# zhvng/open-musiclm

Hardware: NVIDIA H100
Metric: coarse-stage training tokens/sec (positions fed to the transformer per optimiser step / step time) (higher is better)
Workload: dtype bf16 (fp16 operands for the forward GEMMs on LayerNorm outputs x weights; fp32 accumulate)

## Files before the change

### open-musiclm_b200/csrc/attn_bwd_tc.cu

```cuda
#include "common.cuh"
#include "ptx.cuh"
#include "../../include/omlm_b200.h"
#include <stdlib.h>

namespace omlm {

constexpr int kBtThreads = 384;
constexpr int kBtBQ = 64, kBtBK = 128;
constexpr float kBtL2e = 1.4426950408889634f;

constexpr int kBoK = 0, kBoV = 16384, kBoQ = 32768 , kBoDO = 49152 ;
constexpr int kBoP = 65536 , kBoDS = 81920 , kBoBar = 98304 ;
constexpr int kBoSds = 98368;
constexpr int kBtMaxSmem = 232448;
constexpr int kBtSdsLd = 72;
constexpr int kBoWin = kBoSds + 2 * 64 * kBtSdsLd * 4;

static int bt_win_ld(int h) { return ((62 + h) / h + 64 + 23) / 32 * 32 + 8; }

__device__ __forceinline__ float bt_ex2(float x) {
  float y;
  asm("ex2.approx.ftz.f32 %0, %1;" : "=f"(y) : "f"(x));
  return y;
}
__device__ __forceinline__ void bt_red2(float* addr, float a, float b) {
  asm volatile("red.global.add.v2.f32 [%0], {%1, %2};" ::"l"(addr), "f"(a), "f"(b) : "memory");
}

__device__ __forceinline__ int bt_ld_acquire(const int* p) {
  int v;
  asm volatile("ld.acquire.gpu.global.b32 %0, [%1];" : "=r"(v) : "l"(p) : "memory");
  return v;
}
__device__ __forceinline__ unsigned long long bt_globaltimer() {
  unsigned long long t;
  asm volatile("mov.u64 %0, %%globaltimer;" : "=l"(t));
  return t;
}
__device__ __noinline__ void bt_wait_turn(const int* ctr, int turn, int* err) {
  const unsigned long long t0 = bt_globaltimer();
  while (bt_ld_acquire(ctr) != turn) {
    if (*reinterpret_cast<volatile int*>(err) != 0) return;
    if (bt_globaltimer() - t0 > 4000000000ull) { atomicExch(err, 1); return; }
    __nanosleep(64);
  }
}
__device__ __forceinline__ void bt_pass_turn(int* ctr) {
  asm volatile("red.release.gpu.global.add.s32 [%0], 1;" ::"l"(ctr) : "memory");
}

struct BtDet {
  int* turn_dq;
  int* turn_kv;
  int* meta;
  int* err;
  float* dpart;
};

template <bool DET>
__global__ void __launch_bounds__(kBtThreads, 1)
attn_bwd_tc_kernel(const __grid_constant__ CUtensorMap tmQ, const __grid_constant__ CUtensorMap tmDO,
                   const __grid_constant__ CUtensorMap tmKV, const float* __restrict__ lse2, const float* __restrict__ dsum,
                   const float* __restrict__ table, int table_ld, const unsigned char* __restrict__ key_mask,
                   float* __restrict__ dqn, float* __restrict__ dkvn, float* __restrict__ dtable, int N, int h, float scale,
                   int Wacc, int win_ld, int tiles_per_chunk, int nbatch, const BtDet det) {
  extern __shared__ __align__(1024) uint8_t smem_raw[];
  uint8_t* smem = smem_raw + ((1024u - (smem_u32(smem_raw) & 1023u)) & 1023u);
  uint64_t* bars = reinterpret_cast<uint64_t*>(smem + kBoBar);
  uint64_t* kv_full = bars + 0;
  uint64_t* qd_full = bars + 1;
  uint64_t* qd_empty = bars + 3;
  float* dacc = reinterpret_cast<float*>(smem + kBoWin) + 2 * h * win_ld;

  const int wg = threadIdx.x >> 7, lane = threadIdx.x & 31;
  const int R = N * h;
  const int n_rt = (R + kBtBQ - 1) / kBtBQ;
  const int n_kt = (N + kBtBK - 1) / kBtBK;
  const int b = blockIdx.x % nbatch;
  int u = blockIdx.x / nbatch, kt = 0;
  for (; kt < n_kt; ++kt) {
    const int cnt = (n_rt - (kt * kBtBK * h) / kBtBQ + tiles_per_chunk - 1) / tiles_per_chunk;
    if (u < cnt) break;
    u -= cnt;
  }
  const int j0 = kt * kBtBK;
  const int rt0 = (j0 * h) / kBtBQ + u * tiles_per_chunk;
  const int rt1 = min(n_rt, rt0 + tiles_per_chunk);
  const int T = rt1 - rt0;
  const int i_lo = (rt0 * kBtBQ) / h, i_hi = min(N - 1, (rt1 * kBtBQ - 1) / h);
  const int dmin = max(0, i_lo - j0 - (kBtBK - 1));
  const int wacc_used = i_hi - j0 - dmin + 1;

  if (threadIdx.x == 0) {
    tma_prefetch_desc(&tmQ); tma_prefetch_desc(&tmDO); tma_prefetch_desc(&tmKV);
    mbar_init(kv_full, 1);
    for (int i = 0; i < 2; ++i) { mbar_init(&qd_full[i], 1); mbar_init(&qd_empty[i], 2); }
    fence_barrier_init();
  }
  for (int x = threadIdx.x; x < 2 * h * Wacc; x += blockDim.x) dacc[x] = 0.f;
  __syncthreads();

  if (wg == 0) {
    asm volatile("setmaxnreg.dec.sync.aligned.u32 40;");
    if (threadIdx.x == 0) {
      mbar_expect_tx(kv_full, 2 * 16384);
      tma_load_2d(smem + kBoK, &tmKV, kv_full, 0, b * N + j0);
      tma_load_2d(smem + kBoV, &tmKV, kv_full, 64, b * N + j0);
      for (int t = 0; t < T; ++t) {
        const int st = t & 1;
        mbar_wait(&qd_empty[st], ((t >> 1) & 1) ^ 1);
        mbar_expect_tx(&qd_full[st], 2 * 8192);
        tma_load_2d(smem + kBoQ + st * 8192, &tmQ, &qd_full[st], 0, b * R + (rt0 + t) * kBtBQ);
        tma_load_2d(smem + kBoDO + st * 8192, &tmDO, &qd_full[st], 0, b * R + (rt0 + t) * kBtBQ);
      }
    }
  } else {
    asm volatile("setmaxnreg.inc.sync.aligned.u32 232;");
    const int cw = wg - 1;
    const int wq = (threadIdx.x >> 5) & 3, qr = lane >> 2, qc = lane & 3;
    const bool leader = (threadIdx.x & 127) == 0;
    const int kbase = j0 + cw * 64;
    const uint32_t sk = smem_u32(smem + kBoK) + cw * 8192, sv = smem_u32(smem + kBoV) + cw * 8192;
    uint8_t* p_tile = smem + kBoP + cw * 8192;
    uint8_t* ds_tile = smem + kBoDS + cw * 8192;
    float* sdsf = reinterpret_cast<float*>(smem + kBoSds) + cw * 64 * kBtSdsLd;
    float* win = reinterpret_cast<float*>(smem + kBoWin) + cw * h * win_ld;
    float* wacc = dacc + cw * h * Wacc;
    const int tid128 = threadIdx.x & 127;
    const uint32_t sp = smem_u32(p_tile), sds = smem_u32(ds_tile);
    const float sc2 = scale * kBtL2e;
    uint32_t vis = 0;
#pragma unroll
    for (int c = 0; c < 8; ++c)
#pragma unroll
      for (int e = 0; e < 2; ++e) {
        const int j = kbase + 8 * c + 2 * qc + e;
        if (j < N && (key_mask == nullptr || key_mask[static_cast<long long>(b) * N + j] != 0)) vis |= 1u << (2 * c + e);
      }
    float dv[32], dk[32];
#pragma unroll
    for (int x = 0; x < 32; ++x) { dv[x] = 0.f; dk[x] = 0.f; }
    mbar_wait(kv_full, 0);
    for (int t = 0; t < T; ++t) {
      const int st = t & 1;
      const int rbase = (rt0 + t) * kBtBQ;
      const uint32_t sq = smem_u32(smem + kBoQ + st * 8192), sdo = smem_u32(smem + kBoDO + st * 8192);
      mbar_wait(&qd_full[st], (t >> 1) & 1);
      float s[32], dp[32];
      wgmma_fence();
#pragma unroll
      for (int ks = 0; ks < 4; ++ks) {
        Wgmma<64, false>::ss<0, 0>(s, make_smem_desc(sq + ks * 32, 16, 1024), make_smem_desc(sk + ks * 32, 16, 1024), ks > 0 ? 1u : 0u);
        Wgmma<64, false>::ss<0, 0>(dp, make_smem_desc(sdo + ks * 32, 16, 1024), make_smem_desc(sv + ks * 32, 16, 1024), ks > 0 ? 1u : 0u);
      }
      wgmma_commit();
      const int it_lo = min(rbase, R - 1) / h, it_hi = min(rbase + kBtBQ - 1, R - 1) / h;
      {
        const int win_w = it_hi - it_lo + 64, dlo = it_lo - kbase - 63;
        for (int x = tid128; x < h * win_w; x += 128) {
          const int hh = x / win_w, w = x - hh * win_w, d = dlo + w;
          win[hh * win_ld + w] = d >= 0 ? __ldg(table + hh * static_cast<long>(table_ld) + d) * kBtL2e : 0.f;
        }
      }
      asm volatile("bar.sync %0, 128;" ::"r"(1 + cw) : "memory");
      wgmma_wait<0>();
      wgmma_reg_fence(s);
      wgmma_reg_fence(dp);
#pragma unroll
      for (int hr = 0; hr < 2; ++hr) {
        const int lr = wq * 16 + qr + hr * 8;
        const int r = rbase + lr;
        const bool row_ok = r < R;
        const int rc = min(r, R - 1);
        const int i = rc / h, hh = rc - i * h;
        const float lse = lse2[static_cast<long long>(b) * R + rc];
        const float D = dsum[static_cast<long long>(b) * R + rc];
        const float* wrow = win + hh * win_ld + i - it_lo + 63 - 2 * qc;
        const int dcol = i - kbase - 2 * qc;
        uint8_t* prow = p_tile + lr * 128;
        uint8_t* drow = ds_tile + lr * 128;
#pragma unroll
        for (int c = 0; c < 8; ++c) {
          float pp[2], dd[2];
#pragma unroll
          for (int e = 0; e < 2; ++e) {
            const bool live = row_ok && ((vis >> (2 * c + e)) & 1u) && dcol >= 8 * c + e;
            const float x = s[4 * c + 2 * hr + e];
            pp[e] = live ? bt_ex2(fmaf(x, sc2, wrow[-8 * c - e]) - lse) : 0.f;
            dd[e] = pp[e] * (dp[4 * c + 2 * hr + e] - D);
          }
          *reinterpret_cast<float2*>(sdsf + lr * kBtSdsLd + 8 * c + 2 * qc) = make_float2(dd[0], dd[1]);
          const uint32_t off = static_cast<uint32_t>(((c ^ (lr & 7)) << 4) + 4 * qc);
          *reinterpret_cast<uint32_t*>(prow + off) = pack_bf16x2(pp[0], pp[1]);
          *reinterpret_cast<uint32_t*>(drow + off) = pack_bf16x2(dd[0], dd[1]);
        }
      }
      fence_proxy_async();
      asm volatile("bar.sync %0, 128;" ::"r"(1 + cw) : "memory");
      float dq[32];
      wgmma_fence();
#pragma unroll
      for (int ks = 0; ks < 4; ++ks) {
        Wgmma<64, false>::ss<1, 1>(dv, make_smem_desc(sp + ks * 2048, 8192, 1024), make_smem_desc(sdo + ks * 2048, 8192, 1024), 1u);
        Wgmma<64, false>::ss<1, 1>(dk, make_smem_desc(sds + ks * 2048, 8192, 1024), make_smem_desc(sq + ks * 2048, 8192, 1024), 1u);
        Wgmma<64, false>::ss<0, 1>(dq, make_smem_desc(sds + ks * 32, 16, 1024), make_smem_desc(sk + ks * 2048, 8192, 1024), ks > 0 ? 1u : 0u);
      }
      wgmma_commit();
      {
        const int dlo = max(0, it_lo - kbase - 63), dhi = it_hi - kbase;
        const int W = dhi - dlo + 1;
        for (int p = tid128; p < h * W; p += 128) {
          const int hh = p / W, dl = dlo + (p - hh * W);
          const int i0 = max((rbase - hh + h - 1) / h, kbase + dl);
          const int i1 = min(min((rbase + kBtBQ - 1 - hh) / h, N - 1), kbase + dl + 63);
          float sum = 0.f;
          for (int i = i0; i <= i1; ++i) sum += sdsf[(i * h + hh - rbase) * kBtSdsLd + (i - dl - kbase)];
          wacc[hh * Wacc + dl - dmin] += sum;
        }
      }
      wgmma_wait<0>();
      wgmma_reg_fence(dq);
      wgmma_reg_fence(dv);
      wgmma_reg_fence(dk);
      asm volatile("bar.sync %0, 128;" ::"r"(1 + cw) : "memory");
      if (leader) mbar_arrive(&qd_empty[st]);
      int* turn = DET ? det.turn_dq + static_cast<long>(b) * n_rt + rt0 + t : nullptr;
      if constexpr (DET) {
        if (leader) bt_wait_turn(turn, 2 * kt + cw, det.err);
        asm volatile("bar.sync %0, 128;" ::"r"(1 + cw) : "memory");
      }
#pragma unroll
      for (int hr = 0; hr < 2; ++hr) {
        const int r = rbase + wq * 16 + qr + hr * 8;
        if (r < R) {
          float* dst = dqn + (static_cast<long long>(b) * R + r) * 64 + 2 * qc;
#pragma unroll
          for (int c = 0; c < 8; ++c) bt_red2(dst + 8 * c, dq[4 * c + 2 * hr] * scale, dq[4 * c + 2 * hr + 1] * scale);
        }
      }
      if constexpr (DET) {
        __threadfence();
        asm volatile("bar.sync %0, 128;" ::"r"(1 + cw) : "memory");
        if (leader) bt_pass_turn(turn);
      }
    }
    int* kv_turn = DET ? det.turn_kv + (static_cast<long>(b) * n_kt + kt) * 2 + cw : nullptr;
    if constexpr (DET) {
      if (leader) bt_wait_turn(kv_turn, u, det.err);
      asm volatile("bar.sync %0, 128;" ::"r"(1 + cw) : "memory");
    }
#pragma unroll
    for (int hr = 0; hr < 2; ++hr) {
      const int j = kbase + wq * 16 + qr + hr * 8;
      if (j < N) {
        float* dst = dkvn + (static_cast<long long>(b) * N + j) * 128 + 2 * qc;
#pragma unroll
        for (int c = 0; c < 8; ++c) {
          bt_red2(dst + 8 * c, dk[4 * c + 2 * hr] * scale, dk[4 * c + 2 * hr + 1] * scale);
          bt_red2(dst + 64 + 8 * c, dv[4 * c + 2 * hr], dv[4 * c + 2 * hr + 1]);
        }
      }
    }
    if constexpr (DET) {
      __threadfence();
      asm volatile("bar.sync %0, 128;" ::"r"(1 + cw) : "memory");
      if (leader) bt_pass_turn(kv_turn);
    }
    asm volatile("bar.sync 3, 256;" ::: "memory");
    if constexpr (DET) {
      float* up = det.dpart + static_cast<long>(blockIdx.x) * h * Wacc;
      for (int x = threadIdx.x - 128; x < h * wacc_used; x += 256) {
        const int hh = x / wacc_used, w = x - hh * wacc_used;
        up[hh * Wacc + w] = dacc[hh * Wacc + w] + dacc[(h + hh) * Wacc + w];
      }
      if (threadIdx.x == 128) { det.meta[2 * blockIdx.x] = dmin; det.meta[2 * blockIdx.x + 1] = wacc_used; }
    } else {
      for (int x = threadIdx.x - 128; x < h * wacc_used; x += 256) {
        const int hh = x / wacc_used, w = x - hh * wacc_used;
        const float v = dacc[hh * Wacc + w] + dacc[(h + hh) * Wacc + w];
        if (v != 0.f) atomicAdd(dtable + hh * static_cast<long>(table_ld) + dmin + w, v);
      }
    }
  }
}

__global__ void __launch_bounds__(256)
attn_bwd_dtable_reduce_kernel(const float* __restrict__ dpart, const int* __restrict__ meta, int units, int h, int Wacc,
                              float* __restrict__ dtable, int table_ld, int N) {
  const int x = blockIdx.x * blockDim.x + threadIdx.x;
  if (x >= h * N) return;
  const int hh = x / N, d = x - hh * N;
  float* dst = dtable + hh * static_cast<long>(table_ld) + d;
  float acc = *dst;
  for (int u = 0; u < units; ++u) {
    const int w = d - __ldg(meta + 2 * u);
    if (w >= 0 && w < __ldg(meta + 2 * u + 1)) acc += dpart[(static_cast<long>(u) * h + hh) * Wacc + w];
  }
  *dst = acc;
}

__global__ void __launch_bounds__(256)
attn_bwd_tc_dsum_kernel(const __nv_bfloat16* __restrict__ d_o, const __nv_bfloat16* __restrict__ o,
                        float* __restrict__ dsum, long rows, float* __restrict__ dqn, float* __restrict__ dkvn, long kv_vec4) {
  const long tid = static_cast<long>(blockIdx.x) * blockDim.x + threadIdx.x;
  const long r = tid >> 3;
  const int sub = threadIdx.x & 7;
  float s = 0.f;
  for (long i = tid; i < kv_vec4; i += static_cast<long>(gridDim.x) * blockDim.x)
    reinterpret_cast<float4*>(dkvn)[i] = make_float4(0.f, 0.f, 0.f, 0.f);
  if (r < rows) {
    float4* zq = reinterpret_cast<float4*>(dqn + r * 64 + sub * 8);
    zq[0] = make_float4(0.f, 0.f, 0.f, 0.f);
    zq[1] = make_float4(0.f, 0.f, 0.f, 0.f);
    const uint4 a = *reinterpret_cast<const uint4*>(d_o + r * 64 + sub * 8);
    const uint4 bq = *reinterpret_cast<const uint4*>(o + r * 64 + sub * 8);
    const uint32_t aa[4] = {a.x, a.y, a.z, a.w}, bb[4] = {bq.x, bq.y, bq.z, bq.w};
#pragma unroll
    for (int i = 0; i < 4; ++i) {
      const float2 x = unpack_bf16x2(aa[i]), y = unpack_bf16x2(bb[i]);
      s += x.x * y.x + x.y * y.y;
    }
  }
  s += __shfl_xor_sync(0xffffffffu, s, 1);
  s += __shfl_xor_sync(0xffffffffu, s, 2);
  s += __shfl_xor_sync(0xffffffffu, s, 4);
  if (r < rows && sub == 0) dsum[r] = s;
}

}

namespace omlm {

struct BtConfig {
  int tiles_per_chunk, wacc, win_ld, smem_bytes, units_per_batch, n_row_tiles, n_key_tiles;
};

static int bt_config(int B, int N, int heads, BtConfig* cfg) {
  const long R = static_cast<long>(N) * heads;
  const int n_row_tiles = static_cast<int>((R + kBtBQ - 1) / kBtBQ);
  const int n_key_tiles = (N + kBtBK - 1) / kBtBK;
  const int win_ld = bt_win_ld(heads);
  auto wacc_of = [&](int T) { return (T * kBtBQ + heads - 1) / heads + kBtBK + 2; };
  auto smem_of = [&](int T) { return kBoWin + 2 * heads * (win_ld + wacc_of(T)) * 4 + 1024; };
  auto units_of = [&](int T) {
    long units = 0;
    for (int kt = 0; kt < n_key_tiles; ++kt) {
      const int first = (kt * kBtBK * heads) / kBtBQ;
      units += (n_row_tiles - first + T - 1) / T;
    }
    return units;
  };
  OMLM_CHECK_ARG(smem_of(1) <= kBtMaxSmem, "attn_bwd_tc: too many heads (%d) for the shared-memory bias tables", heads);
  int tiles_per_chunk = 1;
  for (int cand = 2; cand <= 2 * n_row_tiles; cand *= 2) {
    const int T = cand < n_row_tiles ? cand : n_row_tiles;
    if (smem_of(T) > kBtMaxSmem) break;
    tiles_per_chunk = T;
    if ((T >= 8 && units_of(T) * B <= 4L * num_sms()) || T == n_row_tiles) break;
  }
  if (const char* e = getenv("OMLM_ATTN_BWD_T")) {
    const int T = atoi(e);
    if (T >= 1 && T <= n_row_tiles && smem_of(T) <= kBtMaxSmem) tiles_per_chunk = T;
  }
  cfg->tiles_per_chunk = tiles_per_chunk;
  cfg->wacc = wacc_of(tiles_per_chunk);
  cfg->win_ld = win_ld;
  cfg->smem_bytes = smem_of(tiles_per_chunk);
  cfg->units_per_batch = static_cast<int>(units_of(tiles_per_chunk));
  cfg->n_row_tiles = n_row_tiles;
  cfg->n_key_tiles = n_key_tiles;
  return 0;
}

static int bt_ints(int B, const BtConfig& c) {
  return B * c.n_row_tiles + 2 * B * c.n_key_tiles + 2 * B * c.units_per_batch + 1;
}

static int attn_bwd_tc_impl(const void* qn, const void* kvn, const void* d_o, const void* o, const float* lse2,
                            const float* table, int table_ld, const unsigned char* key_mask, float* dsum_scratch,
                            float* dqn, float* dkvn, float* dtable, int B, int N, int heads, float scale, bool det,
                            float* ws, long ws_bytes, int* iws, long iws_count, void* stream) {
  OMLM_CHECK_ARG(B > 0 && N > 0 && heads > 0, "attn_bwd_tc: bad shape");
  OMLM_CHECK_ARG(table_ld >= N, "attn_bwd_tc: bias table shorter than the sequence");
  auto st = reinterpret_cast<cudaStream_t>(stream);
  const long R = static_cast<long>(N) * heads;
  const long rows = static_cast<long>(B) * R;
  BtConfig cfg;
  int rc = bt_config(B, N, heads, &cfg);
  if (rc) return rc;
  const int units = B * cfg.units_per_batch;
  BtDet dp{nullptr, nullptr, nullptr, nullptr, nullptr};
  if (det) {
    OMLM_CHECK_ARG(ws != nullptr && iws != nullptr && ws_bytes >= static_cast<long>(units) * heads * cfg.wacc * 4 &&
                   iws_count >= bt_ints(B, cfg), "attn_bwd_tc_det: workspace too small (see omlm_attn_bwd_tc_det_workspace)");
    dp.turn_dq = iws;
    dp.turn_kv = iws + static_cast<long>(B) * cfg.n_row_tiles;
    dp.meta = dp.turn_kv + 2L * B * cfg.n_key_tiles;
    dp.err = iws + iws_count - 1;
    dp.dpart = ws;
    OMLM_CUDA(cudaMemsetAsync(iws, 0, (static_cast<long>(B) * cfg.n_row_tiles + 2L * B * cfg.n_key_tiles) * sizeof(int), st));
  }
  OMLM_KLAUNCH((attn_bwd_tc_dsum_kernel), static_cast<int>((rows * 8 + 255) / 256), 256, 0, st,
      reinterpret_cast<const __nv_bfloat16*>(d_o), reinterpret_cast<const __nv_bfloat16*>(o), dsum_scratch, rows,
      dqn, dkvn, static_cast<long>(B) * N * 128 / 4);
  OMLM_LAUNCH_CHECK();
  CUtensorMap tmQ, tmDO, tmKV;
  rc = make_tmap_bf16_2d(&tmQ, qn, 64, static_cast<uint64_t>(rows), 128, 64, kBtBQ);
  if (rc) return rc;
  rc = make_tmap_bf16_2d(&tmDO, d_o, 64, static_cast<uint64_t>(rows), 128, 64, kBtBQ);
  if (rc) return rc;
  rc = make_tmap_bf16_2d(&tmKV, kvn, 128, static_cast<uint64_t>(B) * N, 256, 64, kBtBK);
  if (rc) return rc;
  auto kern = det ? attn_bwd_tc_kernel<true> : attn_bwd_tc_kernel<false>;
  static int configured[2] = {0, 0};
  if (configured[det] < cfg.smem_bytes) {
    OMLM_CUDA(cudaFuncSetAttribute(kern, cudaFuncAttributeMaxDynamicSharedMemorySize, cfg.smem_bytes));
    configured[det] = cfg.smem_bytes;
  }
  OMLM_KLAUNCH((kern), units, kBtThreads, cfg.smem_bytes, st,
      tmQ, tmDO, tmKV, lse2, dsum_scratch, table, table_ld, key_mask, dqn, dkvn, dtable, N, heads, scale,
      cfg.wacc, cfg.win_ld, cfg.tiles_per_chunk, B, dp);
  OMLM_LAUNCH_CHECK();
  if (det) {
    OMLM_KLAUNCH((attn_bwd_dtable_reduce_kernel), (heads * N + 255) / 256, 256, 0, st,
        static_cast<const float*>(dp.dpart), static_cast<const int*>(dp.meta), units, heads, cfg.wacc, dtable, table_ld, N);
    OMLM_LAUNCH_CHECK();
  }
  return 0;
}

}

extern "C" int omlm_attn_bwd_tc(const void* qn, const void* kvn, const void* d_o, const void* o, const float* lse2,
                                const float* table, int table_ld, const unsigned char* key_mask, float* dsum_scratch,
                                float* dqn, float* dkvn, float* dtable, int B, int N, int heads,
                                float scale, void* stream) {
  return omlm::attn_bwd_tc_impl(qn, kvn, d_o, o, lse2, table, table_ld, key_mask, dsum_scratch, dqn, dkvn, dtable, B, N, heads,
                                scale, false, nullptr, 0, nullptr, 0, stream);
}

extern "C" int omlm_attn_bwd_tc_det(const void* qn, const void* kvn, const void* d_o, const void* o, const float* lse2,
                                    const float* table, int table_ld, const unsigned char* key_mask, float* dsum_scratch,
                                    float* dqn, float* dkvn, float* dtable, int B, int N, int heads, float scale,
                                    float* ws, long ws_bytes, int* iws, long iws_count, void* stream) {
  return omlm::attn_bwd_tc_impl(qn, kvn, d_o, o, lse2, table, table_ld, key_mask, dsum_scratch, dqn, dkvn, dtable, B, N, heads,
                                scale, true, ws, ws_bytes, iws, iws_count, stream);
}

extern "C" int omlm_attn_bwd_tc_det_workspace(int B, int N, int heads, long* ws_bytes, long* iws_count) {
  using namespace omlm;
  OMLM_CHECK_ARG(B > 0 && N > 0 && heads > 0 && ws_bytes != nullptr && iws_count != nullptr, "attn_bwd_tc_det_workspace: bad arguments");
  BtConfig cfg;
  const int rc = bt_config(B, N, heads, &cfg);
  if (rc) return rc;
  *ws_bytes = static_cast<long>(B) * cfg.units_per_batch * heads * cfg.wacc * 4;
  *iws_count = bt_ints(B, cfg);
  return 0;
}
```

### open-musiclm_b200/csrc/ptx.cuh

```cuda
#pragma once
#include <cuda_runtime.h>
#include <cuda_bf16.h>
#include <cuda.h>
#include <stdint.h>

namespace omlm {

__device__ __forceinline__ uint32_t smem_u32(const void* p) {
  return static_cast<uint32_t>(__cvta_generic_to_shared(p));
}
__device__ __forceinline__ uint32_t lane_id() { return threadIdx.x & 31; }

__device__ __forceinline__ bool elect_one() {
  uint32_t pred;
  asm volatile(
      "{\n\t.reg .pred p;\n\t"
      "elect.sync _|p, 0xffffffff;\n\t"
      "selp.u32 %0, 1, 0, p;\n\t}"
      : "=r"(pred));
  return pred != 0;
}

__device__ __forceinline__ void mbar_init(uint64_t* bar, uint32_t count) {
  asm volatile("mbarrier.init.shared::cta.b64 [%0], %1;" ::"r"(smem_u32(bar)), "r"(count));
}
__device__ __forceinline__ void fence_barrier_init() {
  asm volatile("fence.mbarrier_init.release.cluster;" ::: "memory");
}
__device__ __forceinline__ void fence_proxy_async() {
  asm volatile("fence.proxy.async.shared::cta;" ::: "memory");
}
__device__ __forceinline__ void mbar_expect_tx(uint64_t* bar, uint32_t bytes) {
  asm volatile("mbarrier.arrive.expect_tx.shared::cta.b64 _, [%0], %1;" ::"r"(smem_u32(bar)),
               "r"(bytes)
               : "memory");
}
__device__ __forceinline__ void mbar_arrive(uint64_t* bar) {
  asm volatile("mbarrier.arrive.shared::cta.b64 _, [%0];" ::"r"(smem_u32(bar)) : "memory");
}
__device__ __forceinline__ void mbar_wait(uint64_t* bar, uint32_t parity) {
  asm volatile(
      "{\n\t.reg .pred p;\n\t"
      "WAIT_LOOP:\n\t"
      "mbarrier.try_wait.parity.shared::cta.b64 p, [%0], %1;\n\t"
      "@p bra DONE;\n\t"
      "bra WAIT_LOOP;\n\t"
      "DONE:\n\t}"
      ::"r"(smem_u32(bar)), "r"(parity)
      : "memory");
}

__device__ __forceinline__ void tma_prefetch_desc(const CUtensorMap* m) {
  asm volatile("prefetch.tensormap [%0];" ::"l"(reinterpret_cast<uint64_t>(m)) : "memory");
}
__device__ __forceinline__ void tma_load_2d(void* smem_dst, const CUtensorMap* m, uint64_t* bar,
                                            int32_t c0, int32_t c1) {
  asm volatile(
      "cp.async.bulk.tensor.2d.shared::cluster.global.mbarrier::complete_tx::bytes"
      " [%0], [%1, {%3, %4}], [%2];"
      ::"r"(smem_u32(smem_dst)), "l"(reinterpret_cast<uint64_t>(m)), "r"(smem_u32(bar)), "r"(c0),
      "r"(c1)
      : "memory");
}
__device__ __forceinline__ void tma_store_2d(const CUtensorMap* m, const void* smem_src, int32_t c0,
                                             int32_t c1) {
  asm volatile("cp.async.bulk.tensor.2d.global.shared::cta.bulk_group [%0, {%2, %3}], [%1];"
               ::"l"(reinterpret_cast<uint64_t>(m)), "r"(smem_u32(smem_src)), "r"(c0), "r"(c1)
               : "memory");
}
__device__ __forceinline__ void tma_store_3d(const CUtensorMap* m, const void* smem_src, int32_t c0, int32_t c1,
                                             int32_t c2) {
  asm volatile("cp.async.bulk.tensor.3d.global.shared::cta.bulk_group [%0, {%2, %3, %4}], [%1];"
               ::"l"(reinterpret_cast<uint64_t>(m)), "r"(smem_u32(smem_src)), "r"(c0), "r"(c1), "r"(c2)
               : "memory");
}
__device__ __forceinline__ void tma_store_commit() {
  asm volatile("cp.async.bulk.commit_group;" ::: "memory");
}
__device__ __forceinline__ void tma_store_wait_all() {
  asm volatile("cp.async.bulk.wait_group 0;" ::: "memory");
}
template <int N>
__device__ __forceinline__ void tma_store_wait_read() {
  asm volatile("cp.async.bulk.wait_group.read %0;" ::"n"(N) : "memory");
}

__device__ __forceinline__ void wgmma_fence() { asm volatile("wgmma.fence.sync.aligned;" ::: "memory"); }
__device__ __forceinline__ void wgmma_commit() { asm volatile("wgmma.commit_group.sync.aligned;" ::: "memory"); }
template <int N>
__device__ __forceinline__ void wgmma_wait() { asm volatile("wgmma.wait_group.sync.aligned %0;" ::"n"(N) : "memory"); }
template <int R>
__device__ __forceinline__ void wgmma_reg_fence(float (&d)[R]) {
#pragma unroll
  for (int i = 0; i < R; ++i) asm volatile("" : "+f"(d[i])::"memory");
}

__device__ __forceinline__ uint64_t make_smem_desc(uint32_t smem_addr, uint32_t lbo_bytes,
                                                   uint32_t sbo_bytes) {
  uint64_t d = 0;
  d |= static_cast<uint64_t>((smem_addr & 0x3FFFF) >> 4);
  d |= static_cast<uint64_t>((lbo_bytes >> 4) & 0x3FFF) << 16;
  d |= static_cast<uint64_t>((sbo_bytes >> 4) & 0x3FFF) << 32;
  d |= static_cast<uint64_t>(1) << 62;
  return d;
}

template <int N, bool F16> struct Wgmma;
template <> struct Wgmma<64, false> {
  template <int TA, int TB>
  static __device__ __forceinline__ void ss(float (&d)[32], uint64_t a, uint64_t b, uint32_t scale_d) {
    asm volatile(
        "{\n.reg .pred p;\nsetp.ne.b32 p, %34, 0;\n"
        "wgmma.mma_async.sync.aligned.m64n64k16.f32.bf16.bf16 {%0,%1,%2,%3,%4,%5,%6,%7,%8,%9,%10,%11,%12,%13,%14,%15,%16,%17,%18,%19,%20,%21,%22,%23,%24,%25,%26,%27,%28,%29,%30,%31}, %32, %33, p, 1, 1, %35, %36;\n}\n"
        : "+f"(d[0]), "+f"(d[1]), "+f"(d[2]), "+f"(d[3]), "+f"(d[4]), "+f"(d[5]), "+f"(d[6]), "+f"(d[7]), "+f"(d[8]), "+f"(d[9]), "+f"(d[10]), "+f"(d[11]), "+f"(d[12]), "+f"(d[13]), "+f"(d[14]), "+f"(d[15]), "+f"(d[16]), "+f"(d[17]), "+f"(d[18]), "+f"(d[19]), "+f"(d[20]), "+f"(d[21]), "+f"(d[22]), "+f"(d[23]), "+f"(d[24]), "+f"(d[25]), "+f"(d[26]), "+f"(d[27]), "+f"(d[28]), "+f"(d[29]), "+f"(d[30]), "+f"(d[31])
        : "l"(a), "l"(b), "r"(scale_d), "n"(TA), "n"(TB));
  }
  template <int TB>
  static __device__ __forceinline__ void rs(float (&d)[32], const uint32_t (&a)[4], uint64_t b, uint32_t scale_d) {
    asm volatile(
        "{\n.reg .pred p;\nsetp.ne.b32 p, %37, 0;\n"
        "wgmma.mma_async.sync.aligned.m64n64k16.f32.bf16.bf16 {%0,%1,%2,%3,%4,%5,%6,%7,%8,%9,%10,%11,%12,%13,%14,%15,%16,%17,%18,%19,%20,%21,%22,%23,%24,%25,%26,%27,%28,%29,%30,%31}, {%32,%33,%34,%35}, %36, p, 1, 1, %38;\n}\n"
        : "+f"(d[0]), "+f"(d[1]), "+f"(d[2]), "+f"(d[3]), "+f"(d[4]), "+f"(d[5]), "+f"(d[6]), "+f"(d[7]), "+f"(d[8]), "+f"(d[9]), "+f"(d[10]), "+f"(d[11]), "+f"(d[12]), "+f"(d[13]), "+f"(d[14]), "+f"(d[15]), "+f"(d[16]), "+f"(d[17]), "+f"(d[18]), "+f"(d[19]), "+f"(d[20]), "+f"(d[21]), "+f"(d[22]), "+f"(d[23]), "+f"(d[24]), "+f"(d[25]), "+f"(d[26]), "+f"(d[27]), "+f"(d[28]), "+f"(d[29]), "+f"(d[30]), "+f"(d[31])
        : "r"(a[0]), "r"(a[1]), "r"(a[2]), "r"(a[3]), "l"(b), "r"(scale_d), "n"(TB));
  }
};
template <> struct Wgmma<64, true> {
  template <int TA, int TB>
  static __device__ __forceinline__ void ss(float (&d)[32], uint64_t a, uint64_t b, uint32_t scale_d) {
    asm volatile(
        "{\n.reg .pred p;\nsetp.ne.b32 p, %34, 0;\n"
        "wgmma.mma_async.sync.aligned.m64n64k16.f32.f16.f16 {%0,%1,%2,%3,%4,%5,%6,%7,%8,%9,%10,%11,%12,%13,%14,%15,%16,%17,%18,%19,%20,%21,%22,%23,%24,%25,%26,%27,%28,%29,%30,%31}, %32, %33, p, 1, 1, %35, %36;\n}\n"
        : "+f"(d[0]), "+f"(d[1]), "+f"(d[2]), "+f"(d[3]), "+f"(d[4]), "+f"(d[5]), "+f"(d[6]), "+f"(d[7]), "+f"(d[8]), "+f"(d[9]), "+f"(d[10]), "+f"(d[11]), "+f"(d[12]), "+f"(d[13]), "+f"(d[14]), "+f"(d[15]), "+f"(d[16]), "+f"(d[17]), "+f"(d[18]), "+f"(d[19]), "+f"(d[20]), "+f"(d[21]), "+f"(d[22]), "+f"(d[23]), "+f"(d[24]), "+f"(d[25]), "+f"(d[26]), "+f"(d[27]), "+f"(d[28]), "+f"(d[29]), "+f"(d[30]), "+f"(d[31])
        : "l"(a), "l"(b), "r"(scale_d), "n"(TA), "n"(TB));
  }
  template <int TB>
  static __device__ __forceinline__ void rs(float (&d)[32], const uint32_t (&a)[4], uint64_t b, uint32_t scale_d) {
    asm volatile(
        "{\n.reg .pred p;\nsetp.ne.b32 p, %37, 0;\n"
        "wgmma.mma_async.sync.aligned.m64n64k16.f32.f16.f16 {%0,%1,%2,%3,%4,%5,%6,%7,%8,%9,%10,%11,%12,%13,%14,%15,%16,%17,%18,%19,%20,%21,%22,%23,%24,%25,%26,%27,%28,%29,%30,%31}, {%32,%33,%34,%35}, %36, p, 1, 1, %38;\n}\n"
        : "+f"(d[0]), "+f"(d[1]), "+f"(d[2]), "+f"(d[3]), "+f"(d[4]), "+f"(d[5]), "+f"(d[6]), "+f"(d[7]), "+f"(d[8]), "+f"(d[9]), "+f"(d[10]), "+f"(d[11]), "+f"(d[12]), "+f"(d[13]), "+f"(d[14]), "+f"(d[15]), "+f"(d[16]), "+f"(d[17]), "+f"(d[18]), "+f"(d[19]), "+f"(d[20]), "+f"(d[21]), "+f"(d[22]), "+f"(d[23]), "+f"(d[24]), "+f"(d[25]), "+f"(d[26]), "+f"(d[27]), "+f"(d[28]), "+f"(d[29]), "+f"(d[30]), "+f"(d[31])
        : "r"(a[0]), "r"(a[1]), "r"(a[2]), "r"(a[3]), "l"(b), "r"(scale_d), "n"(TB));
  }
};
template <> struct Wgmma<128, false> {
  template <int TA, int TB>
  static __device__ __forceinline__ void ss(float (&d)[64], uint64_t a, uint64_t b, uint32_t scale_d) {
    asm volatile(
        "{\n.reg .pred p;\nsetp.ne.b32 p, %66, 0;\n"
        "wgmma.mma_async.sync.aligned.m64n128k16.f32.bf16.bf16 {%0,%1,%2,%3,%4,%5,%6,%7,%8,%9,%10,%11,%12,%13,%14,%15,%16,%17,%18,%19,%20,%21,%22,%23,%24,%25,%26,%27,%28,%29,%30,%31,%32,%33,%34,%35,%36,%37,%38,%39,%40,%41,%42,%43,%44,%45,%46,%47,%48,%49,%50,%51,%52,%53,%54,%55,%56,%57,%58,%59,%60,%61,%62,%63}, %64, %65, p, 1, 1, %67, %68;\n}\n"
        : "+f"(d[0]), "+f"(d[1]), "+f"(d[2]), "+f"(d[3]), "+f"(d[4]), "+f"(d[5]), "+f"(d[6]), "+f"(d[7]), "+f"(d[8]), "+f"(d[9]), "+f"(d[10]), "+f"(d[11]), "+f"(d[12]), "+f"(d[13]), "+f"(d[14]), "+f"(d[15]), "+f"(d[16]), "+f"(d[17]), "+f"(d[18]), "+f"(d[19]), "+f"(d[20]), "+f"(d[21]), "+f"(d[22]), "+f"(d[23]), "+f"(d[24]), "+f"(d[25]), "+f"(d[26]), "+f"(d[27]), "+f"(d[28]), "+f"(d[29]), "+f"(d[30]), "+f"(d[31]), "+f"(d[32]), "+f"(d[33]), "+f"(d[34]), "+f"(d[35]), "+f"(d[36]), "+f"(d[37]), "+f"(d[38]), "+f"(d[39]), "+f"(d[40]), "+f"(d[41]), "+f"(d[42]), "+f"(d[43]), "+f"(d[44]), "+f"(d[45]), "+f"(d[46]), "+f"(d[47]), "+f"(d[48]), "+f"(d[49]), "+f"(d[50]), "+f"(d[51]), "+f"(d[52]), "+f"(d[53]), "+f"(d[54]), "+f"(d[55]), "+f"(d[56]), "+f"(d[57]), "+f"(d[58]), "+f"(d[59]), "+f"(d[60]), "+f"(d[61]), "+f"(d[62]), "+f"(d[63])
        : "l"(a), "l"(b), "r"(scale_d), "n"(TA), "n"(TB));
  }
};
template <> struct Wgmma<128, true> {
  template <int TA, int TB>
  static __device__ __forceinline__ void ss(float (&d)[64], uint64_t a, uint64_t b, uint32_t scale_d) {
    asm volatile(
        "{\n.reg .pred p;\nsetp.ne.b32 p, %66, 0;\n"
        "wgmma.mma_async.sync.aligned.m64n128k16.f32.f16.f16 {%0,%1,%2,%3,%4,%5,%6,%7,%8,%9,%10,%11,%12,%13,%14,%15,%16,%17,%18,%19,%20,%21,%22,%23,%24,%25,%26,%27,%28,%29,%30,%31,%32,%33,%34,%35,%36,%37,%38,%39,%40,%41,%42,%43,%44,%45,%46,%47,%48,%49,%50,%51,%52,%53,%54,%55,%56,%57,%58,%59,%60,%61,%62,%63}, %64, %65, p, 1, 1, %67, %68;\n}\n"
        : "+f"(d[0]), "+f"(d[1]), "+f"(d[2]), "+f"(d[3]), "+f"(d[4]), "+f"(d[5]), "+f"(d[6]), "+f"(d[7]), "+f"(d[8]), "+f"(d[9]), "+f"(d[10]), "+f"(d[11]), "+f"(d[12]), "+f"(d[13]), "+f"(d[14]), "+f"(d[15]), "+f"(d[16]), "+f"(d[17]), "+f"(d[18]), "+f"(d[19]), "+f"(d[20]), "+f"(d[21]), "+f"(d[22]), "+f"(d[23]), "+f"(d[24]), "+f"(d[25]), "+f"(d[26]), "+f"(d[27]), "+f"(d[28]), "+f"(d[29]), "+f"(d[30]), "+f"(d[31]), "+f"(d[32]), "+f"(d[33]), "+f"(d[34]), "+f"(d[35]), "+f"(d[36]), "+f"(d[37]), "+f"(d[38]), "+f"(d[39]), "+f"(d[40]), "+f"(d[41]), "+f"(d[42]), "+f"(d[43]), "+f"(d[44]), "+f"(d[45]), "+f"(d[46]), "+f"(d[47]), "+f"(d[48]), "+f"(d[49]), "+f"(d[50]), "+f"(d[51]), "+f"(d[52]), "+f"(d[53]), "+f"(d[54]), "+f"(d[55]), "+f"(d[56]), "+f"(d[57]), "+f"(d[58]), "+f"(d[59]), "+f"(d[60]), "+f"(d[61]), "+f"(d[62]), "+f"(d[63])
        : "l"(a), "l"(b), "r"(scale_d), "n"(TA), "n"(TB));
  }
};
template <> struct Wgmma<256, false> {
  template <int TA, int TB>
  static __device__ __forceinline__ void ss(float (&d)[128], uint64_t a, uint64_t b, uint32_t scale_d) {
    asm volatile(
        "{\n.reg .pred p;\nsetp.ne.b32 p, %130, 0;\n"
        "wgmma.mma_async.sync.aligned.m64n256k16.f32.bf16.bf16 {%0,%1,%2,%3,%4,%5,%6,%7,%8,%9,%10,%11,%12,%13,%14,%15,%16,%17,%18,%19,%20,%21,%22,%23,%24,%25,%26,%27,%28,%29,%30,%31,%32,%33,%34,%35,%36,%37,%38,%39,%40,%41,%42,%43,%44,%45,%46,%47,%48,%49,%50,%51,%52,%53,%54,%55,%56,%57,%58,%59,%60,%61,%62,%63,%64,%65,%66,%67,%68,%69,%70,%71,%72,%73,%74,%75,%76,%77,%78,%79,%80,%81,%82,%83,%84,%85,%86,%87,%88,%89,%90,%91,%92,%93,%94,%95,%96,%97,%98,%99,%100,%101,%102,%103,%104,%105,%106,%107,%108,%109,%110,%111,%112,%113,%114,%115,%116,%117,%118,%119,%120,%121,%122,%123,%124,%125,%126,%127}, %128, %129, p, 1, 1, %131, %132;\n}\n"
        : "+f"(d[0]), "+f"(d[1]), "+f"(d[2]), "+f"(d[3]), "+f"(d[4]), "+f"(d[5]), "+f"(d[6]), "+f"(d[7]), "+f"(d[8]), "+f"(d[9]), "+f"(d[10]), "+f"(d[11]), "+f"(d[12]), "+f"(d[13]), "+f"(d[14]), "+f"(d[15]), "+f"(d[16]), "+f"(d[17]), "+f"(d[18]), "+f"(d[19]), "+f"(d[20]), "+f"(d[21]), "+f"(d[22]), "+f"(d[23]), "+f"(d[24]), "+f"(d[25]), "+f"(d[26]), "+f"(d[27]), "+f"(d[28]), "+f"(d[29]), "+f"(d[30]), "+f"(d[31]), "+f"(d[32]), "+f"(d[33]), "+f"(d[34]), "+f"(d[35]), "+f"(d[36]), "+f"(d[37]), "+f"(d[38]), "+f"(d[39]), "+f"(d[40]), "+f"(d[41]), "+f"(d[42]), "+f"(d[43]), "+f"(d[44]), "+f"(d[45]), "+f"(d[46]), "+f"(d[47]), "+f"(d[48]), "+f"(d[49]), "+f"(d[50]), "+f"(d[51]), "+f"(d[52]), "+f"(d[53]), "+f"(d[54]), "+f"(d[55]), "+f"(d[56]), "+f"(d[57]), "+f"(d[58]), "+f"(d[59]), "+f"(d[60]), "+f"(d[61]), "+f"(d[62]), "+f"(d[63]), "+f"(d[64]), "+f"(d[65]), "+f"(d[66]), "+f"(d[67]), "+f"(d[68]), "+f"(d[69]), "+f"(d[70]), "+f"(d[71]), "+f"(d[72]), "+f"(d[73]), "+f"(d[74]), "+f"(d[75]), "+f"(d[76]), "+f"(d[77]), "+f"(d[78]), "+f"(d[79]), "+f"(d[80]), "+f"(d[81]), "+f"(d[82]), "+f"(d[83]), "+f"(d[84]), "+f"(d[85]), "+f"(d[86]), "+f"(d[87]), "+f"(d[88]), "+f"(d[89]), "+f"(d[90]), "+f"(d[91]), "+f"(d[92]), "+f"(d[93]), "+f"(d[94]), "+f"(d[95]), "+f"(d[96]), "+f"(d[97]), "+f"(d[98]), "+f"(d[99]), "+f"(d[100]), "+f"(d[101]), "+f"(d[102]), "+f"(d[103]), "+f"(d[104]), "+f"(d[105]), "+f"(d[106]), "+f"(d[107]), "+f"(d[108]), "+f"(d[109]), "+f"(d[110]), "+f"(d[111]), "+f"(d[112]), "+f"(d[113]), "+f"(d[114]), "+f"(d[115]), "+f"(d[116]), "+f"(d[117]), "+f"(d[118]), "+f"(d[119]), "+f"(d[120]), "+f"(d[121]), "+f"(d[122]), "+f"(d[123]), "+f"(d[124]), "+f"(d[125]), "+f"(d[126]), "+f"(d[127])
        : "l"(a), "l"(b), "r"(scale_d), "n"(TA), "n"(TB));
  }
};
template <> struct Wgmma<256, true> {
  template <int TA, int TB>
  static __device__ __forceinline__ void ss(float (&d)[128], uint64_t a, uint64_t b, uint32_t scale_d) {
    asm volatile(
        "{\n.reg .pred p;\nsetp.ne.b32 p, %130, 0;\n"
        "wgmma.mma_async.sync.aligned.m64n256k16.f32.f16.f16 {%0,%1,%2,%3,%4,%5,%6,%7,%8,%9,%10,%11,%12,%13,%14,%15,%16,%17,%18,%19,%20,%21,%22,%23,%24,%25,%26,%27,%28,%29,%30,%31,%32,%33,%34,%35,%36,%37,%38,%39,%40,%41,%42,%43,%44,%45,%46,%47,%48,%49,%50,%51,%52,%53,%54,%55,%56,%57,%58,%59,%60,%61,%62,%63,%64,%65,%66,%67,%68,%69,%70,%71,%72,%73,%74,%75,%76,%77,%78,%79,%80,%81,%82,%83,%84,%85,%86,%87,%88,%89,%90,%91,%92,%93,%94,%95,%96,%97,%98,%99,%100,%101,%102,%103,%104,%105,%106,%107,%108,%109,%110,%111,%112,%113,%114,%115,%116,%117,%118,%119,%120,%121,%122,%123,%124,%125,%126,%127}, %128, %129, p, 1, 1, %131, %132;\n}\n"
        : "+f"(d[0]), "+f"(d[1]), "+f"(d[2]), "+f"(d[3]), "+f"(d[4]), "+f"(d[5]), "+f"(d[6]), "+f"(d[7]), "+f"(d[8]), "+f"(d[9]), "+f"(d[10]), "+f"(d[11]), "+f"(d[12]), "+f"(d[13]), "+f"(d[14]), "+f"(d[15]), "+f"(d[16]), "+f"(d[17]), "+f"(d[18]), "+f"(d[19]), "+f"(d[20]), "+f"(d[21]), "+f"(d[22]), "+f"(d[23]), "+f"(d[24]), "+f"(d[25]), "+f"(d[26]), "+f"(d[27]), "+f"(d[28]), "+f"(d[29]), "+f"(d[30]), "+f"(d[31]), "+f"(d[32]), "+f"(d[33]), "+f"(d[34]), "+f"(d[35]), "+f"(d[36]), "+f"(d[37]), "+f"(d[38]), "+f"(d[39]), "+f"(d[40]), "+f"(d[41]), "+f"(d[42]), "+f"(d[43]), "+f"(d[44]), "+f"(d[45]), "+f"(d[46]), "+f"(d[47]), "+f"(d[48]), "+f"(d[49]), "+f"(d[50]), "+f"(d[51]), "+f"(d[52]), "+f"(d[53]), "+f"(d[54]), "+f"(d[55]), "+f"(d[56]), "+f"(d[57]), "+f"(d[58]), "+f"(d[59]), "+f"(d[60]), "+f"(d[61]), "+f"(d[62]), "+f"(d[63]), "+f"(d[64]), "+f"(d[65]), "+f"(d[66]), "+f"(d[67]), "+f"(d[68]), "+f"(d[69]), "+f"(d[70]), "+f"(d[71]), "+f"(d[72]), "+f"(d[73]), "+f"(d[74]), "+f"(d[75]), "+f"(d[76]), "+f"(d[77]), "+f"(d[78]), "+f"(d[79]), "+f"(d[80]), "+f"(d[81]), "+f"(d[82]), "+f"(d[83]), "+f"(d[84]), "+f"(d[85]), "+f"(d[86]), "+f"(d[87]), "+f"(d[88]), "+f"(d[89]), "+f"(d[90]), "+f"(d[91]), "+f"(d[92]), "+f"(d[93]), "+f"(d[94]), "+f"(d[95]), "+f"(d[96]), "+f"(d[97]), "+f"(d[98]), "+f"(d[99]), "+f"(d[100]), "+f"(d[101]), "+f"(d[102]), "+f"(d[103]), "+f"(d[104]), "+f"(d[105]), "+f"(d[106]), "+f"(d[107]), "+f"(d[108]), "+f"(d[109]), "+f"(d[110]), "+f"(d[111]), "+f"(d[112]), "+f"(d[113]), "+f"(d[114]), "+f"(d[115]), "+f"(d[116]), "+f"(d[117]), "+f"(d[118]), "+f"(d[119]), "+f"(d[120]), "+f"(d[121]), "+f"(d[122]), "+f"(d[123]), "+f"(d[124]), "+f"(d[125]), "+f"(d[126]), "+f"(d[127])
        : "l"(a), "l"(b), "r"(scale_d), "n"(TA), "n"(TB));
  }
};

}
```

Before: 575,000.

## Offload dQ ordered reduction and LSE/dsum loads to producer warps in attention backward

Splits the producer warpgroup into specialised warps. One warp issues TMA loads, one stages lse2 and dsum into shared memory per tile, and, in deterministic mode, two warps perform the turn-ordered dQ reduction via bulk async reduce from a shared staging buffer. Consumers now hand dQ off through new mbarriers instead of spinning on the turn counter themselves. The bias-gradient window reduction is also restructured to process two items per thread with 8-wide unrolled strided sums. This adds barrier handshakes and reuses the sdsf buffer for dQ staging, which risks hazards on that buffer.

```diff
diff --git a/open-musiclm_b200/csrc/attn_bwd_tc.cu b/open-musiclm_b200/csrc/attn_bwd_tc.cu
--- a/open-musiclm_b200/csrc/attn_bwd_tc.cu
+++ b/open-musiclm_b200/csrc/attn_bwd_tc.cu
@@ -11,7 +11,8 @@
 
 constexpr int kBoK = 0, kBoV = 16384, kBoQ = 32768 , kBoDO = 49152 ;
 constexpr int kBoP = 65536 , kBoDS = 81920 , kBoBar = 98304 ;
-constexpr int kBoSds = 98368;
+constexpr int kBoLs = 98432;
+constexpr int kBoSds = 99456;
 constexpr int kBtMaxSmem = 232448;
 constexpr int kBtSdsLd = 72;
 constexpr int kBoWin = kBoSds + 2 * 64 * kBtSdsLd * 4;
@@ -37,7 +38,7 @@
   asm volatile("mov.u64 %0, %%globaltimer;" : "=l"(t));
   return t;
 }
-__device__ __noinline__ void bt_wait_turn(const int* ctr, int turn, int* err) {
+__device__ __forceinline__ void bt_wait_turn(const int* ctr, int turn, int* err) {
   const unsigned long long t0 = bt_globaltimer();
   while (bt_ld_acquire(ctr) != turn) {
     if (*reinterpret_cast<volatile int*>(err) != 0) return;
@@ -70,6 +71,9 @@
   uint64_t* kv_full = bars + 0;
   uint64_t* qd_full = bars + 1;
   uint64_t* qd_empty = bars + 3;
+  uint64_t* dq_full = bars + 5;
+  uint64_t* dq_empty = bars + 7;
+  float* sls = reinterpret_cast<float*>(smem + kBoLs);
   float* dacc = reinterpret_cast<float*>(smem + kBoWin) + 2 * h * win_ld;
 
   const int wg = threadIdx.x >> 7, lane = threadIdx.x & 31;
@@ -94,24 +98,69 @@
   if (threadIdx.x == 0) {
     tma_prefetch_desc(&tmQ); tma_prefetch_desc(&tmDO); tma_prefetch_desc(&tmKV);
     mbar_init(kv_full, 1);
-    for (int i = 0; i < 2; ++i) { mbar_init(&qd_full[i], 1); mbar_init(&qd_empty[i], 2); }
+    for (int i = 0; i < 2; ++i) {
+      mbar_init(&qd_full[i], 2);
+      mbar_init(&qd_empty[i], 2);
+      mbar_init(&dq_full[i], 128);
+      mbar_init(&dq_empty[i], 1);
+    }
     fence_barrier_init();
+    mbar_expect_tx(kv_full, 2 * 16384);
+    tma_load_2d(smem + kBoK, &tmKV, kv_full, 0, b * N + j0);
+    tma_load_2d(smem + kBoV, &tmKV, kv_full, 64, b * N + j0);
   }
   for (int x = threadIdx.x; x < 2 * h * Wacc; x += blockDim.x) dacc[x] = 0.f;
   __syncthreads();
 
   if (wg == 0) {
     asm volatile("setmaxnreg.dec.sync.aligned.u32 40;");
-    if (threadIdx.x == 0) {
-      mbar_expect_tx(kv_full, 2 * 16384);
-      tma_load_2d(smem + kBoK, &tmKV, kv_full, 0, b * N + j0);
-      tma_load_2d(smem + kBoV, &tmKV, kv_full, 64, b * N + j0);
+    const int pw = threadIdx.x >> 5;
+    if (pw == 0) {
+      if (lane == 0) {
+        for (int t = 0; t < T; ++t) {
+          const int st = t & 1;
+          mbar_wait(&qd_empty[st], ((t >> 1) & 1) ^ 1);
+          mbar_expect_tx(&qd_full[st], 2 * 8192);
+          tma_load_2d(smem + kBoQ + st * 8192, &tmQ, &qd_full[st], 0, b * R + (rt0 + t) * kBtBQ);
+          tma_load_2d(smem + kBoDO + st * 8192, &tmDO, &qd_full[st], 0, b * R + (rt0 + t) * kBtBQ);
+        }
+      }
+    } else if (pw == 1) {
       for (int t = 0; t < T; ++t) {
         const int st = t & 1;
+        const int rbase = (rt0 + t) * kBtBQ;
         mbar_wait(&qd_empty[st], ((t >> 1) & 1) ^ 1);
-        mbar_expect_tx(&qd_full[st], 2 * 8192);
-        tma_load_2d(smem + kBoQ + st * 8192, &tmQ, &qd_full[st], 0, b * R + (rt0 + t) * kBtBQ);
-        tma_load_2d(smem + kBoDO + st * 8192, &tmDO, &qd_full[st], 0, b * R + (rt0 + t) * kBtBQ);
+#pragma unroll
+        for (int k = lane; k < kBtBQ; k += 32) {
+          const long long r = static_cast<long long>(b) * R + min(rbase + k, R - 1);
+          sls[st * 128 + k] = lse2[r];
+          sls[st * 128 + 64 + k] = dsum[r];
+        }
+        __syncwarp();
+        if (lane == 0) mbar_arrive(&qd_full[st]);
+      }
+    } else if (DET) {
+      const int cw = pw - 2;
+      const float* sq_f = reinterpret_cast<const float*>(smem + kBoSds) + cw * 64 * kBtSdsLd;
+      for (int t = 0; t < T; ++t) {
+        const int rbase = (rt0 + t) * kBtBQ;
+        mbar_wait(&dq_full[cw], t & 1);
+        int* turn = det.turn_dq + static_cast<long>(b) * n_rt + rt0 + t;
+        if (lane == 0) bt_wait_turn(turn, 2 * kt + cw, det.err);
+        __syncwarp();
+        fence_proxy_async_global();
+#pragma unroll
+        for (int k = lane; k < kBtBQ; k += 32)
+          if (rbase + k < R) bulk_reduce_add_f32(dqn + (static_cast<long long>(b) * R + rbase + k) * 64, sq_f + k * kBtSdsLd, 256);
+        tma_store_commit();
+        tma_store_wait_all();
+        fence_proxy_async_global();
+        __threadfence();
+        __syncwarp();
+        if (lane == 0) {
+          bt_pass_turn(turn);
+          mbar_arrive(&dq_empty[cw]);
+        }
       }
     }
   } else {
@@ -145,6 +194,7 @@
       const int st = t & 1;
       const int rbase = (rt0 + t) * kBtBQ;
       const uint32_t sq = smem_u32(smem + kBoQ + st * 8192), sdo = smem_u32(smem + kBoDO + st * 8192);
+      const float* tls = sls + st * 128;
       mbar_wait(&qd_full[st], (t >> 1) & 1);
       float s[32], dp[32];
       wgmma_fence();
@@ -166,6 +216,7 @@
       wgmma_wait<0>();
       wgmma_reg_fence(s);
       wgmma_reg_fence(dp);
+      if (DET && t > 0) mbar_wait(&dq_empty[cw], (t - 1) & 1);
 #pragma unroll
       for (int hr = 0; hr < 2; ++hr) {
         const int lr = wq * 16 + qr + hr * 8;
@@ -173,8 +224,8 @@
         const bool row_ok = r < R;
         const int rc = min(r, R - 1);
         const int i = rc / h, hh = rc - i * h;
-        const float lse = lse2[static_cast<long long>(b) * R + rc];
-        const float D = dsum[static_cast<long long>(b) * R + rc];
+        const float lse = tls[lr];
+        const float D = tls[64 + lr];
         const float* wrow = win + hh * win_ld + i - it_lo + 63 - 2 * qc;
         const int dcol = i - kbase - 2 * qc;
         uint8_t* prow = p_tile + lr * 128;
@@ -209,13 +260,46 @@
       {
         const int dlo = max(0, it_lo - kbase - 63), dhi = it_hi - kbase;
         const int W = dhi - dlo + 1;
-        for (int p = tid128; p < h * W; p += 128) {
-          const int hh = p / W, dl = dlo + (p - hh * W);
-          const int i0 = max((rbase - hh + h - 1) / h, kbase + dl);
-          const int i1 = min(min((rbase + kBtBQ - 1 - hh) / h, N - 1), kbase + dl + 63);
-          float sum = 0.f;
-          for (int i = i0; i <= i1; ++i) sum += sdsf[(i * h + hh - rbase) * kBtSdsLd + (i - dl - kbase)];
-          wacc[hh * Wacc + dl - dmin] += sum;
+        const int q0 = rbase / h, r0 = rbase - q0 * h;
+        const int q1 = (rbase + kBtBQ - 1) / h, r1 = rbase + kBtBQ - 1 - q1 * h;
+        const int step = h * kBtSdsLd + 1;
+        for (int p = tid128; p < h * W; p += 256) {
+          int n[2];
+          const float* src[2];
+          float* dst[2];
+#pragma unroll
+          for (int u = 0; u < 2; ++u) {
+            const int pu = p + 128 * u;
+            n[u] = 0;
+            src[u] = sdsf;
+            dst[u] = nullptr;
+            if (pu < h * W) {
+              const int hh = pu / W, dl = dlo + (pu - hh * W);
+              const int i0 = max(q0 + (hh < r0 ? 1 : 0), kbase + dl);
+              const int i1 = min(min(q1 - (hh > r1 ? 1 : 0), N - 1), kbase + dl + 63);
+              n[u] = i1 - i0 + 1;
+              if (n[u] > 0) src[u] = sdsf + (i0 * h + hh - rbase) * kBtSdsLd + (i0 - dl - kbase);
+              dst[u] = wacc + hh * Wacc + dl - dmin;
+            }
+          }
+          float sum[2] = {0.f, 0.f};
+          for (int k0 = 0; k0 < max(n[0], n[1]); k0 += 8) {
+            float v[2][8];
+#pragma unroll
+            for (int u = 0; u < 2; ++u)
+#pragma unroll
+              for (int k = 0; k < 8; ++k) {
+                const float x = src[u][max(min(k0 + k, n[u] - 1), 0) * step];
+                v[u][k] = k0 + k < n[u] ? x : 0.f;
+              }
+#pragma unroll
+            for (int u = 0; u < 2; ++u)
+#pragma unroll
+              for (int k = 0; k < 8; ++k) sum[u] += v[u][k];
+          }
+#pragma unroll
+          for (int u = 0; u < 2; ++u)
+            if (dst[u] != nullptr) *dst[u] += sum[u];
         }
       }
       wgmma_wait<0>();
@@ -224,24 +308,26 @@
       wgmma_reg_fence(dk);
       asm volatile("bar.sync %0, 128;" ::"r"(1 + cw) : "memory");
       if (leader) mbar_arrive(&qd_empty[st]);
-      int* turn = DET ? det.turn_dq + static_cast<long>(b) * n_rt + rt0 + t : nullptr;
       if constexpr (DET) {
-        if (leader) bt_wait_turn(turn, 2 * kt + cw, det.err);
-        asm volatile("bar.sync %0, 128;" ::"r"(1 + cw) : "memory");
-      }
-#pragma unroll
-      for (int hr = 0; hr < 2; ++hr) {
-        const int r = rbase + wq * 16 + qr + hr * 8;
-        if (r < R) {
-          float* dst = dqn + (static_cast<long long>(b) * R + r) * 64 + 2 * qc;
-#pragma unroll
-          for (int c = 0; c < 8; ++c) bt_red2(dst + 8 * c, dq[4 * c + 2 * hr] * scale, dq[4 * c + 2 * hr + 1] * scale);
-        }
-      }
-      if constexpr (DET) {
-        __threadfence();
-        asm volatile("bar.sync %0, 128;" ::"r"(1 + cw) : "memory");
-        if (leader) bt_pass_turn(turn);
+#pragma unroll
+        for (int hr = 0; hr < 2; ++hr) {
+          const int lr = wq * 16 + qr + hr * 8;
+#pragma unroll
+          for (int c = 0; c < 8; ++c)
+            *reinterpret_cast<float2*>(sdsf + lr * kBtSdsLd + 8 * c + 2 * qc) = make_float2(dq[4 * c + 2 * hr] * scale, dq[4 * c + 2 * hr + 1] * scale);
+        }
+        fence_proxy_async();
+        mbar_arrive(&dq_full[cw]);
+      } else {
+#pragma unroll
+        for (int hr = 0; hr < 2; ++hr) {
+          const int r = rbase + wq * 16 + qr + hr * 8;
+          if (r < R) {
+            float* dst = dqn + (static_cast<long long>(b) * R + r) * 64 + 2 * qc;
+#pragma unroll
+            for (int c = 0; c < 8; ++c) bt_red2(dst + 8 * c, dq[4 * c + 2 * hr] * scale, dq[4 * c + 2 * hr + 1] * scale);
+          }
+        }
       }
     }
     int* kv_turn = DET ? det.turn_kv + (static_cast<long>(b) * n_kt + kt) * 2 + cw : nullptr;
diff --git a/open-musiclm_b200/csrc/ptx.cuh b/open-musiclm_b200/csrc/ptx.cuh
--- a/open-musiclm_b200/csrc/ptx.cuh
+++ b/open-musiclm_b200/csrc/ptx.cuh
@@ -83,6 +83,14 @@
 template <int N>
 __device__ __forceinline__ void tma_store_wait_read() {
   asm volatile("cp.async.bulk.wait_group.read %0;" ::"n"(N) : "memory");
+}
+__device__ __forceinline__ void bulk_reduce_add_f32(float* gdst, const void* smem_src, uint32_t bytes) {
+  asm volatile("cp.reduce.async.bulk.global.shared::cta.bulk_group.add.f32 [%0], [%1], %2;"
+               ::"l"(gdst), "r"(smem_u32(smem_src)), "r"(bytes)
+               : "memory");
+}
+__device__ __forceinline__ void fence_proxy_async_global() {
+  asm volatile("fence.proxy.async.global;" ::: "memory");
 }
 
 __device__ __forceinline__ void wgmma_fence() { asm volatile("wgmma.fence.sync.aligned;" ::: "memory"); }
```

Measured after the change: 581,500 (median of 6 runs). +1.1%, better.
